# topling/toplingdb

Hardware: NVIDIA H100
Metric: compaction_input_kv_MB_per_s (higher is better)
Workload: dtype u8

## Files before the change

toplingdb_b200/csrc/encode.cu:

```cuda
#include "bloom_rules.h"
#include "common.cuh"
#include "gp_rules.h"
#include "kernels.h"
#include "scan.cuh"

namespace b200c {

constexpr int kTT = kEncTile;
constexpr int kW = kEncTile + kEncHalo;
constexpr int kEncThreads = 256;

__global__ void __launch_bounds__(256)
encode_sizes_kernel(KeyCols m, const unsigned long long* __restrict__ n_dev, uint32_t* __restrict__ esz, uint8_t* __restrict__ eshared,
                    TileStat* __restrict__ tstat, unsigned long long* __restrict__ tprefix, uint32_t* __restrict__ min_s1) {
  const uint64_t n = *n_dev;
  const uint64_t ntiles = (n + kEncTile - 1) / kEncTile;
  uint32_t mn = 0xffffffffu, mxs = 0;
  __shared__ unsigned long long red[5];
  __shared__ uint32_t s_mn, s_mx;
  if (threadIdx.x == 0) {
    s_mn = 0xffffffffu;
    s_mx = 0;
  }
  for (uint64_t tile = blockIdx.x; tile < ntiles; tile += gridDim.x) {
    if (threadIdx.x < 5) red[threadIdx.x] = threadIdx.x == 3 ? ~0ull : 0ull;
    __syncthreads();
    const uint64_t t0 = tile * kEncTile, t1 = (t0 + kEncTile) < n ? (t0 + kEncTile) : n;
    unsigned long long kb = 0, vb = 0, nd = 0, smin = ~0ull, smax = 0;
    constexpr int kB = 4;
    for (uint64_t ib = t0; ib < t1; ib += (uint64_t)kB * blockDim.x) {
      ulonglong2 c[kB], pc[kB];
      uint64_t ctr[kB], ptr_[kB];
      uint32_t cm[kB], pm[kB];
      const unsigned lane = threadIdx.x & 31;
#pragma unroll
      for (int q = 0; q < kB; q++) {
        const uint64_t i = ib + (uint64_t)q * blockDim.x + threadIdx.x;
        c[q] = make_ulonglong2(0, 0);
        pc[q] = make_ulonglong2(0, 0);
        ctr[q] = ptr_[q] = 0;
        cm[q] = pm[q] = 0;
        if (i < t1) {
          c[q] = m.pfx[i];
          ctr[q] = m.tr[i];
          cm[q] = m.meta[i];
          if (lane == 0 && i > 0) {
            pc[q] = m.pfx[i - 1];
            ptr_[q] = m.tr[i - 1];
            pm[q] = m.meta[i - 1];
          }
        }
      }
#pragma unroll
      for (int q = 0; q < kB; q++) {
        const uint64_t i = ib + (uint64_t)q * blockDim.x + threadIdx.x;
        const uint64_t nx = __shfl_up_sync(0xffffffffu, c[q].x, 1), ny = __shfl_up_sync(0xffffffffu, c[q].y, 1);
        const uint64_t nt = __shfl_up_sync(0xffffffffu, ctr[q], 1);
        const uint32_t nm = __shfl_up_sync(0xffffffffu, cm[q], 1);
        if (lane != 0) {
          pc[q] = make_ulonglong2(nx, ny);
          ptr_[q] = nt;
          pm[q] = nm;
        }
        if (i < t1) {
          const uint32_t ulen = meta_ulen(cm[q]), vs = meta_vlen(cm[q]), ks = ulen + 8;
          const uint32_t sh = i > 0 ? shared_prefix(c[q].x, c[q].y, ulen, ctr[q], pc[q].x, pc[q].y, meta_ulen(pm[q]), ptr_[q]) : 0;
          const uint32_t s1 = entry_size(sh, ks, vs);
          esz[i] = s1;
          eshared[i] = (uint8_t)sh;
          mn = s1 < mn ? s1 : mn;
          mxs = s1 > mxs ? s1 : mxs;
          kb += ks;
          vb += vs;
          nd += is_deletion_type((uint32_t)(ctr[q] & 0xff));
          const uint64_t sq = ctr[q] >> 8;
          smin = sq < smin ? sq : smin;
          smax = sq > smax ? sq : smax;
        }
      }
    }
#pragma unroll
    for (int d = 16; d; d >>= 1) {
      kb += __shfl_xor_sync(0xffffffffu, kb, d);
      vb += __shfl_xor_sync(0xffffffffu, vb, d);
      nd += __shfl_xor_sync(0xffffffffu, nd, d);
      const unsigned long long a = __shfl_xor_sync(0xffffffffu, smin, d), b = __shfl_xor_sync(0xffffffffu, smax, d);
      smin = a < smin ? a : smin;
      smax = b > smax ? b : smax;
    }
    if ((threadIdx.x & 31) == 0) {
      atomicAdd(&red[0], kb);
      atomicAdd(&red[1], vb);
      atomicAdd(&red[2], nd);
      atomicMin(&red[3], smin);
      atomicMax(&red[4], smax);
    }
    __syncthreads();
    if (threadIdx.x == 0) {
      tstat[tile] = TileStat{red[0], red[1], red[2], red[3], red[4]};
      tprefix[tile] = t1;
    }
    __syncthreads();
  }
  mn = __reduce_min_sync(0xffffffffu, mn);
  mxs = __reduce_max_sync(0xffffffffu, mxs);
  __syncthreads();
  if ((threadIdx.x & 31) == 0) {
    atomicMin(&s_mn, mn);
    atomicMax(&s_mx, mxs);
  }
  __syncthreads();
  if (threadIdx.x == 0 && s_mn != 0xffffffffu) {
    atomicMin(min_s1, s_mn);
    atomicMax(min_s1 + 1, s_mx);
  }
}

template <typename PT>
struct Window {
  PT P[kW + 1];
  uint32_t Q[kW];
  uint64_t ws[33];
  uint32_t wlen;
  uint32_t at_end;
  uint32_t smax;
};

template <typename PT>
__device__ void build_window(Window<PT>& w, const KeyCols& m, const uint32_t* esz, const uint8_t* eshared, uint64_t n, uint64_t tile,
                             uint32_t R) {
  const uint64_t wstart = tile * (uint64_t)kTT;
  const uint32_t wlen = (uint32_t)((n - wstart) < (uint64_t)kW ? (n - wstart) : (uint64_t)kW);
  uint32_t mx = 0;
  if (threadIdx.x == 0) w.smax = 0;
  constexpr int kBatch = 8;
  for (uint32_t jb = 0; jb < wlen; jb += kBatch * kEncThreads) {
    uint32_t s1v[kBatch], shv[kBatch], mtv[kBatch];
#pragma unroll
    for (int i = 0; i < kBatch; i++) {
      const uint32_t j = jb + i * kEncThreads + threadIdx.x;
      s1v[i] = shv[i] = mtv[i] = 0;
      if (j < wlen) {
        s1v[i] = esz[wstart + j];
        shv[i] = eshared[wstart + j];
        mtv[i] = m.meta[wstart + j];
      }
    }
#pragma unroll
    for (int i = 0; i < kBatch; i++) {
      const uint32_t j = jb + i * kEncThreads + threadIdx.x;
      if (j < wlen) {
        const uint32_t sh = shv[i], ks = meta_ulen(mtv[i]) + 8;
        const uint32_t d = 1u + varint_len32(ks) + sh - varint_len32(sh) - varint_len32(ks - sh);
        w.Q[j] = d;
        w.P[j + 1] = (PT)s1v[i];
        mx = s1v[i] + d > mx ? s1v[i] + d : mx;
      }
    }
  }
  __syncthreads();
  constexpr int kPer = ((kW + kEncThreads - 1) / kEncThreads) | 1;
  const uint32_t j0 = threadIdx.x * kPer;
  uint64_t loc[kPer], sum = 0;
#pragma unroll
  for (int i = 0; i < kPer; i++) {
    const uint32_t j = j0 + i;
    loc[i] = j < wlen ? w.P[j + 1] : 0;
    sum += loc[i];
  }
#pragma unroll
  for (int d = 16; d; d >>= 1) {
    uint32_t o = __shfl_xor_sync(0xffffffffu, mx, d);
    mx = o > mx ? o : mx;
  }
  uint64_t ex = block_excl_scan64(sum, nullptr, w.ws);
  if ((threadIdx.x & 31) == 0) atomicMax(&w.smax, mx);
#pragma unroll
  for (int i = 0; i < kPer; i++) {
    uint32_t j = j0 + i;
    if (j <= wlen && j <= (uint32_t)kW) w.P[j] = (PT)ex;
    ex += loc[i];
  }
  if (threadIdx.x == 0) {
    w.wlen = wlen;
    w.at_end = (wstart + wlen == n);
  }
  __syncthreads();
  if ((R & (R - 1)) == 0 && R <= 32 && kEncThreads % R == 0) {
    const uint32_t c = threadIdx.x & (R - 1), part = threadIdx.x / R, nparts = kEncThreads / R;
    const uint32_t per_class = (wlen + R - 1) / R;
    const uint32_t chunk = (per_class + nparts - 1) / nparts;
    const uint32_t first = part * chunk;
    uint32_t sum = 0;
    for (uint32_t i = 0; i < chunk; i++) {
      const uint32_t j = c + R * (first + i);
      if (j < wlen) sum += w.Q[j];
    }
    __shared__ uint32_t part_sum[kEncThreads];
    part_sum[threadIdx.x] = sum;
    __syncthreads();
    uint32_t run = 0;
    for (uint32_t q = 0; q < part; q++) run += part_sum[c + R * q];
    for (uint32_t i = 0; i < chunk; i++) {
      const uint32_t j = c + R * (first + i);
      if (j < wlen) {
        run += w.Q[j];
        w.Q[j] = run;
      }
    }
    __syncthreads();
  } else {
    for (uint32_t off = R; off < wlen; off <<= 1) {
      uint32_t add[kPer];
#pragma unroll
      for (int i = 0; i < kPer; i++) {
        uint32_t j = j0 + i;
        add[i] = (j < wlen && j >= off) ? w.Q[j - off] : 0;
      }
      __syncthreads();
#pragma unroll
      for (int i = 0; i < kPer; i++) {
        uint32_t j = j0 + i;
        if (j < wlen) w.Q[j] += add[i];
      }
      __syncthreads();
    }
  }
}

struct CutParams {
  uint32_t BS, LIM, R, rshift;
};
__host__ __device__ __forceinline__ CutParams make_cut(uint32_t bs, uint32_t lim, uint32_t r) {
  CutParams c{bs, lim, r, 32};
  if ((r & (r - 1)) == 0) {
    uint32_t sft = 0;
    while ((1u << sft) < r) sft++;
    c.rshift = sft;
  }
  return c;
}
__device__ __forceinline__ uint32_t div_r(uint32_t x, const CutParams& cp) { return cp.rshift < 32 ? x >> cp.rshift : x / cp.R; }
template <typename PT>
struct BlockStart {
  uint32_t a;
  PT pa;
  uint32_t qa;
};
template <typename PT>
__device__ __forceinline__ BlockStart<PT> block_start(const Window<PT>& w, uint32_t a, const CutParams& cp) {
  BlockStart<PT> s;
  s.a = a;
  s.pa = w.P[a];
  s.qa = a >= cp.R ? w.Q[a - cp.R] : 0u;
  return s;
}
template <typename PT>
__device__ __forceinline__ PT blk_payload(const Window<PT>& w, const BlockStart<PT>& s, uint32_t b, const CutParams& cp) {
  const uint32_t nrm1 = div_r(b - 1 - s.a, cp);
  const uint32_t last = s.a + cp.R * nrm1;
  const uint32_t q = w.Q[last] - s.qa;
  return (PT)(w.P[b] - s.pa) + (PT)q + (PT)(4u * (nrm1 + 1) + 4u);
}
template <typename PT>
__device__ __forceinline__ PT blk_payload(const Window<PT>& w, uint32_t a, uint32_t b, const CutParams& cp) {
  return blk_payload(w, block_start(w, a, cp), b, cp);
}
template <typename PT>
__device__ __forceinline__ uint32_t next_block(const Window<PT>& w, uint32_t a, const CutParams& cp, uint32_t hint, PT* pay_out) {
  const uint32_t wlen = w.wlen;
  const BlockStart<PT> bs = block_start(w, a, cp);
  PT thr = (PT)(cp.BS - 1);
  if (cp.LIM) {
    thr = (PT)cp.LIM;
    const uint64_t guard = (uint64_t)w.smax + 7;
    if (cp.BS > guard && cp.BS - guard - 1 > thr) thr = (PT)(cp.BS - guard - 1);
  }
  uint32_t lo = a + 1, hi = wlen + 1;
  PT ec_hi = 0;
  if (hint > a + 1 && hint <= wlen) {
    const PT ph = blk_payload(w, bs, hint, cp);
    uint32_t step = 1;
    if (ph > thr) {
      hi = hint;
      ec_hi = ph;
      while (hi - lo >= step) {
        const uint32_t mid = hi - step;
        const PT pm = blk_payload(w, bs, mid, cp);
        if (pm > thr) {
          hi = mid;
          ec_hi = pm;
          step <<= 1;
        } else {
          lo = mid + 1;
          break;
        }
      }
    } else {
      lo = hint + 1;
      while (lo + step - 1 <= wlen) {
        const uint32_t mid = lo + step - 1;
        const PT pm = blk_payload(w, bs, mid, cp);
        if (pm > thr) {
          hi = mid;
          ec_hi = pm;
          break;
// ... 6 lines not shown
  while (lo < hi) {
    const uint32_t mid = (lo + hi) >> 1;
    const PT pm = blk_payload(w, bs, mid, cp);
    if (pm > thr) {
      hi = mid;
      ec_hi = pm;
    } else {
      lo = mid + 1;
    }
  }
  if (lo >= wlen) {
    if (!w.at_end) return 0xffffffffu;
    *pay_out = blk_payload(w, bs, wlen, cp);
    return wlen;
  }
  PT ec = ec_hi;
  uint32_t m = lo - a;
  uint32_t mr = cp.rshift < 32 ? (m & (cp.R - 1)) : (m % cp.R);
  for (uint32_t b = lo; b < wlen; b++) {
    if (ec >= cp.BS) {
      *pay_out = ec;
      return b;
    }
    const PT s1 = (PT)(w.P[b + 1] - w.P[b]);
    const bool at_restart = mr == 0;
    const PT d = at_restart ? (PT)(w.Q[b] - (b >= cp.R ? w.Q[b - cp.R] : 0u)) : (PT)0;
    if (cp.LIM) {
      const PT dfull = at_restart ? d : (PT)(w.Q[b] - (b >= cp.R ? w.Q[b - cp.R] : 0u));
      if (ec + s1 + dfull + 3 + (at_restart ? 4 : 0) > cp.BS) {
        *pay_out = ec;
        return b;
      }
    }
    ec += s1 + (at_restart ? d + 4 : 0);
    mr = mr + 1 == cp.R ? 0 : mr + 1;
  }
  if (!w.at_end) return 0xffffffffu;
  *pay_out = ec;
  return wlen;
}

constexpr int kEncGroup = kEncGroupTiles;
__device__ __forceinline__ TileRow ldcg_row(const TileRow* p) {
  const uint4 v = __ldcg(reinterpret_cast<const uint4*>(p));
  TileRow r;
  r.exit = v.x;
  r.nblk = v.y;
  r.bytes = (uint64_t)v.z | ((uint64_t)v.w << 32);
  return r;
}
static_assert(sizeof(TileRow) == 16, "TileRow is moved as one 16-byte vector");
__device__ void compose_group(const EncodeWork& wk, uint64_t n, uint64_t g, uint64_t t0, uint64_t t1, uint32_t hc) {
  const uint64_t gstart = t0 * (uint64_t)kTT;
  for (uint32_t c = threadIdx.x; c < hc; c += blockDim.x) {
    uint64_t x = gstart + c, bytes = 0;
    uint32_t nb = 0;
    bool bad = false;
    for (uint64_t t = t0; t < t1 && x < n; t++) {
      const uint64_t tstart = t * (uint64_t)kTT, tend = (tstart + kTT) < n ? (tstart + kTT) : n;
      if (x >= tend) continue;
      const uint64_t cc = x - tstart;
      if (cc >= hc) {
        bad = true;
        break;
      }
      const TileRow r = ldcg_row(&wk.rows[t * hc + cc]);
      if (r.exit == 0xffffffffu) {
        bad = true;
        break;
      }
      x = tstart + r.exit;
      nb += r.nblk;
      bytes += r.bytes;
    }
    TileRow o;
    o.exit = bad ? 0xffffffffu : (uint32_t)(x - gstart);
    o.nblk = nb;
    o.bytes = bytes;
    wk.grows[g * hc + c] = o;
  }
}

template <typename PT>
struct TablesSmem {
  Window<PT> w;
  uint16_t nxt[kTT];
  uint32_t disk[kTT];
};
template <typename PT>
__global__ void __launch_bounds__(kEncThreads, sizeof(PT) == 4 ? 3 : 2)
encode_tables_kernel(KeyCols m, EncodeParams ep, EncodeWork wk, uint64_t n, uint32_t hc, uint16_t* __restrict__ g_nxt,
                     uint32_t* __restrict__ g_disk, uint32_t* __restrict__ err) {
  extern __shared__ __align__(16) uint8_t smem_raw[];
  TablesSmem<PT>& s = *reinterpret_cast<TablesSmem<PT>*>(smem_raw);
  const uint64_t tile = blockIdx.x, wstart = tile * (uint64_t)kTT;
  const CutParams cp = make_cut(ep.block_size, ep.block_size_limit, ep.restart_interval);
  build_window(s.w, m, wk.esz, wk.eshared, n, tile, cp.R);
  const uint32_t tl = s.w.wlen < (uint32_t)kTT ? s.w.wlen : (uint32_t)kTT;
  {
    constexpr int kPer = kTT / kEncThreads;
    const PT total = s.w.P[s.w.wlen];
    const uint32_t per_block = total ? (uint32_t)(((uint64_t)ep.block_size * s.w.wlen) / total) : 0;
    uint32_t prev_pos = 0, prev_b = 0;
    for (int i = 0; i < kPer; i++) {
      const uint32_t j = threadIdx.x * kPer + ((i + threadIdx.x) & (kPer - 1));
      if (j >= tl) continue;
      uint32_t hint = j + 1 + per_block;
      if (prev_b) hint = prev_b + j - prev_pos;
      if (hint > s.w.wlen) hint = s.w.wlen;
      PT pay = 0;
      uint32_t b = next_block(s.w, j, cp, hint, &pay);
      prev_pos = j;
      prev_b = b == 0xffffffffu ? 0 : b;
      uint16_t nx = 0xffff;
      uint32_t dk = 0;
      if (b != 0xffffffffu) {
        nx = (uint16_t)b;
        const uint64_t pay5 = (uint64_t)pay + 5;
        dk = pay5 > 0xffffffffull ? 0xffffffffu : (uint32_t)pay5;
      }
      s.nxt[j] = nx;
      s.disk[j] = dk;
    }
  }
  __syncthreads();
  for (uint32_t j = threadIdx.x; j < tl; j += kEncThreads) {
    g_nxt[wstart + j] = s.nxt[j];
    g_disk[wstart + j] = s.disk[j];
  }
  __syncthreads();
  for (uint32_t c = threadIdx.x; c < hc; c += kEncThreads) {
    uint32_t x = c, nb = 0;
    uint64_t bytes = 0;
    bool bad = false;
    while (x < tl) {
      uint32_t y = s.nxt[x];
      if (y == 0xffff || y <= x) {
        bad = true;
        break;
      }
      bytes += s.disk[x];
      nb++;
      x = y;
    }
    TileRow r;
    r.exit = bad ? 0xffffffffu : x;
    r.nblk = nb;
    r.bytes = bytes;
    wk.rows[tile * hc + c] = r;
  }
  (void)err;
  __threadfence();
  __syncthreads();
  __shared__ uint32_t s_last;
  const uint64_t g = tile / kEncGroupTiles, ntiles = (n + kTT - 1) / kTT;
  const uint64_t t0 = g * kEncGroupTiles, t1 = (t0 + kEncGroupTiles) < ntiles ? (t0 + kEncGroupTiles) : ntiles;
  if (threadIdx.x == 0) s_last = atomicAdd(&wk.gdone[g], 1u) + 1 == (uint32_t)(t1 - t0);
  __syncthreads();
  if (!s_last) return;
  __threadfence();
  compose_group(wk, n, g, t0, t1, hc);
  __threadfence();
  __syncthreads();
  if (threadIdx.x == 0) atomicExch(&wk.gready[g], 1u);
}

struct WalkState {
  uint64_t a;
  uint64_t blk;
  uint64_t foff;
  uint64_t f_first_entry, f_first_blk;
  uint32_t f;
};
__device__ __forceinline__ void close_file(FileRec* files, WalkState& st, uint64_t end_entry, uint32_t* err) {
  if (files == nullptr) return;
  if (st.f >= kMaxOutFiles) {
    atomicOr(err, kErrInternal);
    return;
  }
  FileRec& fr = files[st.f];
  fr.first_entry = st.f_first_entry;
  fr.n_entries = end_entry - st.f_first_entry;
  fr.first_block = st.f_first_blk;
  fr.n_blocks = st.blk - st.f_first_blk;
  fr.data_size = st.foff;
  fr.index_size = 0;
  fr.raw_key_size = fr.raw_value_size = fr.num_deletions = 0;
  fr.smallest_seq = ~0ull;
  fr.largest_seq = 0;
  fr.index_has_seq = 0;
  fr.filter_entries = fr.filter_bytes = 0;
}
__device__ __forceinline__ uint64_t single_entry_block_bytes(const KeyCols& m, const EncodeWork& wk, uint64_t y) {
  uint32_t sh = wk.eshared[y], ks = meta_ulen(m.meta[y]) + 8;
  uint64_t s0 = (uint64_t)wk.esz[y] + 1u + varint_len32(ks) + sh - varint_len32(sh) - varint_len32(ks - sh);
  return s0 + 4 + 4 + 5;
}
__device__ uint64_t truncated_block_bytes(const KeyCols& m, const EncodeWork& wk, uint32_t R, uint64_t a, uint64_t e) {
  uint64_t sum = 0;
  for (uint64_t j0 = a; j0 < e; j0 += 8) {
    uint32_t s1[8], sh[8], mt[8];
#pragma unroll
    for (int q = 0; q < 8; q++) {
      const uint64_t j = j0 + q;
      s1[q] = sh[q] = mt[q] = 0;
      if (j < e) {
        s1[q] = wk.esz[j];
        sh[q] = wk.eshared[j];
        mt[q] = m.meta[j];
      }
    }
#pragma unroll
    for (int q = 0; q < 8; q++) {
      const uint64_t j = j0 + q;
      if (j < e) {
        sum += s1[q];
        if ((j - a) % R == 0) {
          const uint32_t ks = meta_ulen(mt[q]) + 8;
          sum += 1u + varint_len32(ks) + sh[q] - varint_len32(sh[q]) - varint_len32(ks - sh[q]);
        }
      }
    }
  }
  const uint64_t nrest = (e - a + R - 1) / R;
// ... 184 lines not shown
          const uint64_t cc = st.a - tstart;
          TileRow r;
          r.exit = 0xffffffffu;
          if (cc < hc) r = tcache[(t - cta) * hc + cc];
          const bool table_ok = cc < hc && r.exit != 0xffffffffu;
          const bool cut = !table_ok || (ep.output_level != 0 && st.foff + r.bytes >= ep.max_output_file_size) || tstart + r.exit >= n ||
                           next_ev <= tstart + r.exit;
          if (cut) {
            req = 1;
            req_idx = t;
            break;
          }
          st.a = tstart + r.exit;
          st.blk += r.nblk;
          st.foff += r.bytes;
          continue;
        }
        if (cg >= ngroups) {
          fin = 1;
          break;
        }
        const uint64_t gg = cg, t0 = gg * kEncGroup, gstart = t0 * (uint64_t)kTT;
        const uint64_t t1 = (t0 + kEncGroup) < ntiles ? (t0 + kEncGroup) : ntiles;
        const uint64_t gend = (t1 * (uint64_t)kTT) < n ? (t1 * (uint64_t)kTT) : n;
        if (st.a < gend && !(gg >= cga && gg < cga + cgn)) {
          req = 2;
          req_idx = gg;
          break;
        }
        TileState gs{st.a, st.blk, st.foff, st.f, 0};
        wk.gstate[gg] = gs;
        wk.gflag[gg] = 0;
        cg++;
        if (st.a >= gend) continue;
        const uint64_t cc = st.a - gstart;
        TileRow r;
        r.exit = 0xffffffffu;
        if (cc < hc) r = gcache[(gg - cga) * hc + cc];
        const bool table_ok = cc < hc && r.exit != 0xffffffffu;
        const bool cut = !table_ok || (ep.output_level != 0 && st.foff + r.bytes >= ep.max_output_file_size) || gstart + r.exit >= n ||
                         next_ev <= gstart + r.exit;
        if (cut) {
          wk.gflag[gg] = 1;
          ct = t0;
          ctend = t1;
          continue;
        }
        st.a = gstart + r.exit;
        st.blk += r.nblk;
        st.foff += r.bytes;
      }
      s.st = st;
      s.g = cg;
      s.t = ct;
      s.tend = ctend;
      s.req = req;
      s.req_idx = req_idx;
      if (fin) s.done = 1;
    }
    __syncthreads();
    const uint32_t req = s.req;
    const uint64_t ridx = s.req_idx;
    uint32_t done = s.done;
    if (req == 2 || req == 3) {
      const uint64_t total = req == 2 ? ngroups : s.tend;
      uint32_t cnt = (uint32_t)((total - ridx) < cache_rows ? (total - ridx) : cache_rows);
      if (req == 2) {
        if (threadIdx.x == 0) {
          volatile uint32_t* rdy = wk.gready;
          if (first_wait) {
            unsigned long long t0, t1;
            asm volatile("mov.u64 %0, %globaltimer;" : "=l"(t0));
            while (rdy[ridx] == 0) {
              __nanosleep(256);
              asm volatile("mov.u64 %0, %globaltimer;" : "=l"(t1));
              if (t1 - t0 > timeout_ns) {
                s.done = 2;
                break;
              }
            }
          } else {
            while (rdy[ridx] == 0) __nanosleep(256);
          }
          uint32_t have = 1;
          while (have < cnt && rdy[ridx + have] != 0) have++;
          s.refill = have;
          __threadfence();
        }
        __syncthreads();
        if (s.done == 2) return;
        first_wait = false;
        cnt = s.refill;
      }
      const uint4* src = reinterpret_cast<const uint4*>((req == 2 ? wk.grows : wk.rows) + ridx * hc);
      uint4* dst = reinterpret_cast<uint4*>(req == 2 ? gcache : tcache);
      coop_copy_cg<uint4, 8>(dst, src, cnt * hc);
      if (threadIdx.x == 0) {
        if (req == 2) {
          s.ga = ridx;
          s.gn = cnt;
        } else {
          s.ta = ridx;
          s.tn = cnt;
        }
      }
    } else if (req == 1) {
      const uint64_t tstart = ridx * (uint64_t)kTT;
      const uint32_t tl = (uint32_t)(((tstart + kTT) < n ? (tstart + kTT) : n) - tstart);
      const uint32_t c0 = (uint32_t)(s.st.a > tstart ? (s.st.a - tstart) & ~7ull : 0);
      const uint32_t c1 = (tl + 7u) & ~7u;
      coop_copy_cg<uint4, 4>(reinterpret_cast<uint4*>(s.nxt + c0), reinterpret_cast<const uint4*>(wk.nxt + tstart + c0), (c1 - c0) / 8);
      coop_copy_cg<uint4, 8>(reinterpret_cast<uint4*>(s.disk + c0), reinterpret_cast<const uint4*>(wk.disk + tstart + c0), (c1 - c0) / 4);
      __syncthreads();
      if (ep.gp.n == 0) {
        for (uint32_t i = c0 + threadIdx.x; i < tl; i += blockDim.x) s.nd[i] = ((uint64_t)s.nxt[i] << 32) | s.disk[i];
        __syncthreads();
      }
      if (threadIdx.x == 0) {
        WalkState st = s.st;
        GpState g = s.gp;
        bool chased = true;
        if (ep.gp.n) {
          chased = chase_tile<1>(s.nxt, s.disk, tstart, tl, n, ep, m, wk, st, wk.files, nullptr, 0, err, &g);
        } else {
          const uint32_t nd_base = (uint32_t)__cvta_generic_to_shared(s.nd);
          const uint64_t left = n - tstart;
          const uint32_t nlocal = left < 0xffffull ? (uint32_t)left : 0xffffu;
          const bool cut_files = ep.output_level != 0;
          const uint64_t fmax = ep.max_output_file_size;
          uint32_t x = (uint32_t)(st.a - tstart);
          uint64_t foff = st.foff, blk = st.blk;
          while (x < tl) {
            for (;;) {
              uint64_t v;
              asm volatile("ld.shared.u64 %0, [%1];" : "=l"(v) : "r"(nd_base + 8u * x));
              const uint32_t yr = (uint32_t)(v >> 32), d = (uint32_t)v;
              const uint64_t nf = foff + d;
              if (yr <= x || yr >= nlocal || (cut_files && nf >= fmax)) break;
              foff = nf;
              blk++;
              x = yr;
              if (x >= tl) break;
            }
            if (x >= tl) break;
            st.a = tstart + x;
            st.foff = foff;
            st.blk = blk;
            chased = chase_tile<0>(s.nxt, s.disk, tstart, x + 1, n, ep, m, wk, st, wk.files, nullptr, 0, err);
            if (!chased || st.a >= n) break;
            x = (uint32_t)(st.a - tstart);
            foff = st.foff;
            blk = st.blk;
          }
          if (chased && st.a < n && x >= tl && st.a < tstart + x) {
            st.a = tstart + x;
            st.foff = foff;
            st.blk = blk;
          }
        }
        s.gp = g;
        if (!chased) {
          atomicOr(err, kErrBlockTooLong);
          s.done = 1;
        }
        s.st = st;
      }
      __syncthreads();
      done = s.done;
    }
    __syncthreads();
    if (done) break;
  }
  if (threadIdx.x == 0) {
    wk.totals[0] = s.st.blk;
    wk.totals[1] = s.st.f;
    TileState ts{n, s.st.blk, 0, s.st.f, 0};
    for (uint64_t t = s.t; t < s.tend; t++) wk.tstate[t] = ts;
    for (uint64_t gg = s.g; gg < ngroups; gg++) {
      wk.gstate[gg] = ts;
      wk.gflag[gg] = 0;
    }
    __threadfence();
    if (attempt == 1) atomicExch(sflag, 1u);
  }
}

__global__ void encode_tilestate_kernel(EncodeWork wk, uint64_t n, uint64_t ntiles, uint32_t hc, uint32_t* __restrict__ err) {
  const uint64_t g = blockIdx.x * (uint64_t)blockDim.x + threadIdx.x;
  const uint64_t ngroups = (ntiles + kEncGroup - 1) / kEncGroup;
  if (g >= ngroups || wk.gflag[g]) return;
  const TileState gs = wk.gstate[g];
  uint64_t a = gs.entry, blk = gs.blk, foff = gs.file_off;
  const uint64_t t0 = g * kEncGroup, t1 = (t0 + kEncGroup) < ntiles ? (t0 + kEncGroup) : ntiles;
  for (uint64_t t = t0; t < t1; t++) {
    const uint64_t tstart = t * (uint64_t)kTT, tend = (tstart + kTT) < n ? (tstart + kTT) : n;
    TileState ts{a < n ? a : n, blk, foff, gs.file_idx, 0};
    wk.tstate[t] = ts;
    if (a >= n || a >= tend) continue;
    const uint64_t cc = a - tstart;
    if (cc >= hc) {
      atomicOr(err, kErrBlockTooLong);
      return;
    }
    const TileRow r = wk.rows[t * hc + cc];
    if (r.exit == 0xffffffffu) {
      atomicOr(err, kErrBlockTooLong);
      return;
    }
    a = tstart + r.exit;
    blk += r.nblk;
    foff += r.bytes;
  }
}

struct BlistSmem {
  uint16_t nxt[kTT];
  uint32_t disk[kTT];
  uint8_t is_start[kTT];
  uint64_t ws[33];
  uint32_t serial;
};
__global__ void __launch_bounds__(kEncThreads)
encode_blocklist_kernel(KeyCols m, EncodeParams ep, EncodeWork wk, uint64_t n, uint64_t nblk_cap, uint32_t* __restrict__ err) {
  __shared__ BlistSmem s;
  const uint64_t tile = blockIdx.x, tstart = tile * (uint64_t)kTT;
  const uint64_t tend = (tstart + kTT) < n ? (tstart + kTT) : n;
  const uint32_t tl = (uint32_t)(tend - tstart);
  const TileState ts = wk.tstate[tile];
  if (ts.entry >= tend) return;
  for (uint32_t j = threadIdx.x; j < tl; j += kEncThreads) {
    s.nxt[j] = wk.nxt[tstart + j];
    s.disk[j] = wk.disk[tstart + j];
    s.is_start[j] = 0;
  }
  __syncthreads();
  if (threadIdx.x == 0) {
    uint32_t x = (uint32_t)(ts.entry - tstart);
    uint64_t bytes = 0;
    bool bad = false, ends = false;
    while (x < tl) {
      uint32_t y = s.nxt[x];
      if (y == 0xffff || y <= x) {
        bad = true;
        break;
      }
      s.is_start[x] = 1;
      bytes += s.disk[x];
      if (tstart + y >= n) ends = true;
      x = y;
    }
    if (bad) atomicOr(err, kErrBlockTooLong);
    bool gp_cut = false;
    if (ep.gp.n && !bad) {
      const uint32_t nc = *ep.gp_ncuts;
      uint32_t lo = 0, hi = nc;
      while (lo < hi) {
        const uint32_t mid = (lo + hi) >> 1;
        if (ep.gp_cuts[mid].entry <= ts.entry) lo = mid + 1;
        else hi = mid;
      }
      gp_cut = lo < nc && ep.gp_cuts[lo].entry <= tstart + x;
    }
    s.serial = bad ? 2 : ((ends || gp_cut || (ep.output_level != 0 && ts.file_off + bytes >= ep.max_output_file_size)) ? 1 : 0);
    if (s.serial == 1) {
      WalkState st;
      st.a = ts.entry;
      st.blk = ts.blk;
      st.foff = ts.file_off;
      st.f = ts.file_idx;
      st.f_first_entry = 0;
      st.f_first_blk = 0;
      const bool chased = ep.gp.n ? chase_tile<2>(s.nxt, s.disk, tstart, tl, n, ep, m, wk, st, nullptr, wk.blocks, nblk_cap, err)
                                  : chase_tile<0>(s.nxt, s.disk, tstart, tl, n, ep, m, wk, st, nullptr, wk.blocks, nblk_cap, err);
      if (!chased) atomicOr(err, kErrBlockTooLong);
    }
  }
  __syncthreads();
  if (s.serial != 0) return;
  constexpr int kPer = kTT / kEncThreads;
  const uint32_t j0 = threadIdx.x * kPer;
  uint32_t cnt = 0;
  uint64_t bytes = 0;
#pragma unroll
  for (int i = 0; i < kPer; i++) {
    uint32_t j = j0 + i;
    if (j < tl && s.is_start[j]) {
      cnt++;
      bytes += s.disk[j];
    }
  }
  uint64_t packed = ((uint64_t)cnt << 48) | bytes;
  uint64_t ex = block_excl_scan64(packed, nullptr, s.ws);
  uint64_t r = ts.blk + (ex >> 48), off = ts.file_off + (ex & ((1ull << 48) - 1));
#pragma unroll
  for (int i = 0; i < kPer; i++) {
    uint32_t j = j0 + i;
    if (j < tl && s.is_start[j]) {
      if (r < nblk_cap) wk.blocks[r] = BlockRec{tstart + j, off, ts.file_idx, (uint32_t)(s.nxt[j] - j)};
      r++;
      off += s.disk[j];
    }
  }
}

__device__ __forceinline__ uint64_t index_entries_bytes(const EncodeWork& wk, uint64_t b0, uint64_t nb) {
  return wk.idx_eoff[b0 + nb - 1] + wk.idx_esz[b0 + nb - 1] - wk.idx_eoff[b0];
}

__global__ void encode_filestats_kernel(KeyCols m, EncodeWork wk, uint32_t nfiles) {
  const uint32_t f = blockIdx.x;
  if (f >= nfiles) return;
  const uint64_t f0 = wk.files[f].first_entry, f1 = f0 + wk.files[f].n_entries;
  __shared__ unsigned long long red[5];
  if (threadIdx.x < 5) red[threadIdx.x] = threadIdx.x == 3 ? ~0ull : 0ull;
  __syncthreads();
  const unsigned long long kVal = (1ull << 62) - 1;
// ... 985 lines not shown
                        uint32_t cksum, uint8_t* const* out_base, uint64_t* contrib, const uint64_t* contrib_off, cudaStream_t st) {
  if (n == 0 || nfiles == 0) return;
  const int probes = bloom_num_probes((int)millibits);
  static PerDeviceFlag attr;
  const uint64_t dev_bit = attr.bit_of_current_device();
  const int smem = (int)kBloomSliceBytes + 16 + (kBloomThreads / 32) * kBloomStage * 8;
  if (!attr.is_set(dev_bit)) {
    cudaFuncSetAttribute(bloom_slices_kernel, cudaFuncAttributeMaxDynamicSharedMemorySize, smem);
    attr.set(dev_bit);
  }
  const unsigned slices = (max_filter_bytes + kBloomSliceBytes - 1) / kBloomSliceBytes;
  bloom_slices_kernel<<<dim3(slices ? slices : 1, nfiles), kBloomThreads, smem, st>>>(hashes, files, nfiles, probes, out_base);
  if (cksum == 4) file_block_contrib_kernel<<<dim3(32, nfiles), 256, 0, st>>>(files, nfiles, kFilterBlock, out_base, contrib, contrib_off);
  file_block_trailer_kernel<<<(nfiles + 3) / 4, 128, 0, st>>>(files, nfiles, kFilterBlock, cksum, out_base, contrib, contrib_off);
}

__global__ void gp_rank_kernel(KeyCols m, const GpKey* __restrict__ smallest, const GpKey* __restrict__ largest, uint32_t n,
                               uint64_t* __restrict__ lo, uint64_t* __restrict__ eq, uint64_t* __restrict__ hi) {
  const uint32_t i = blockIdx.x * blockDim.x + threadIdx.x;
  if (i >= n) return;
  auto bound = [&](const GpKey& k, bool upper) -> uint64_t {
    uint64_t a = 0, b = m.n;
    while (a < b) {
      const uint64_t mid = a + ((b - a) >> 1);
      const ulonglong2 p = m.pfx[mid];
      const int c = ukey_cmp(p.x, p.y, meta_ulen(m.meta[mid]), k.hi, k.lo, k.ulen);
      if (c < 0 || (upper && c == 0)) a = mid + 1;
      else b = mid;
    }
    return a;
  };
  lo[i] = bound(smallest[i], false);
  eq[i] = bound(largest[i], false);
  hi[i] = bound(largest[i], true);
}
void launch_gp_ranks(KeyCols m, const GpKey* smallest, const GpKey* largest, uint32_t n, uint64_t* lo, uint64_t* eq, uint64_t* hi,
                     cudaStream_t st) {
  if (n) gp_rank_kernel<<<(n + 63) / 64, 64, 0, st>>>(m, smallest, largest, n, lo, eq, hi);
}

__global__ void scatter_tails_kernel(const TailCopy* __restrict__ recs, const uint8_t* __restrict__ staged, uint8_t* __restrict__ out) {
  const TailCopy r = recs[blockIdx.x];
  for (uint32_t i = threadIdx.x; i < r.len; i += blockDim.x) out[r.dst_off + i] = staged[r.src_off + i];
}

__global__ void gather_small_kernel(const uint64_t* __restrict__ small, uint32_t small_words, const FileRec* __restrict__ files,
                                    const uint64_t* __restrict__ nfiles_dev, uint64_t* __restrict__ dst) {
  const uint32_t t = blockIdx.x * blockDim.x + threadIdx.x, nt = gridDim.x * blockDim.x;
  for (uint32_t i = t; i < small_words; i += nt) dst[i] = small[i];
  if (files) {
    uint64_t n = *nfiles_dev;
    if (n > kMaxOutFiles) n = kMaxOutFiles;
    const uint64_t words = n * (sizeof(FileRec) / 8);
    const uint64_t* src = reinterpret_cast<const uint64_t*>(files);
    for (uint64_t i = t; i < words; i += nt) dst[small_words + i] = src[i];
  }
}
static_assert(sizeof(FileRec) % 8 == 0, "FileRec is copied word-wise");

void launch_gather_small(const uint64_t* small, uint32_t small_bytes, const FileRec* files, const uint64_t* nfiles_dev, uint8_t* dst,
                         cudaStream_t st) {
  gather_small_kernel<<<files ? 8 : 1, 256, 0, st>>>(small, small_bytes / 8, files, nfiles_dev, reinterpret_cast<uint64_t*>(dst));
}
__global__ void copy_small_kernel(const uint8_t* __restrict__ src, uint8_t* __restrict__ dst, uint32_t n) {
  for (uint32_t i = threadIdx.x; i < n; i += blockDim.x) dst[i] = src[i];
}
void launch_copy_small(const void* src, void* dst, uint32_t n, cudaStream_t st) {
  if (n) copy_small_kernel<<<1, 256, 0, st>>>(static_cast<const uint8_t*>(src), static_cast<uint8_t*>(dst), n);
}
void launch_scatter_tails(const TailCopy* recs, uint32_t n, const uint8_t* staged, uint8_t* out, cudaStream_t st) {
  if (n) scatter_tails_kernel<<<n, 256, 0, st>>>(recs, staged, out);
}
void launch_encode_sizes(KeyCols m, const unsigned long long* n_dev, EncodeWork w, unsigned long long* tprefix_out, uint64_t n_cap,
                         int sms, cudaStream_t st) {
  if (n_cap == 0) return;
  const uint64_t tiles = (n_cap + kEncTile - 1) / kEncTile;
  encode_sizes_kernel<<<(unsigned)(tiles < (unsigned)sms * 8 ? tiles : (unsigned)sms * 8), 256, 0, st>>>(m, n_dev, w.esz, w.eshared, w.tstat, tprefix_out, w.min_s1);
}
void launch_encode_tables(KeyCols m, EncodeParams ep, EncodeWork w, uint64_t ntiles, uint32_t hc, uint32_t max_s1, uint32_t* err,
                          cudaStream_t st) {
  if (ntiles == 0) return;
  static PerDeviceFlag attr;
  const uint64_t dev_bit = attr.bit_of_current_device();
  if (!attr.is_set(dev_bit)) {
    cudaFuncSetAttribute(encode_tables_kernel<uint32_t>, cudaFuncAttributeMaxDynamicSharedMemorySize, (int)sizeof(TablesSmem<uint32_t>));
    cudaFuncSetAttribute(encode_tables_kernel<uint64_t>, cudaFuncAttributeMaxDynamicSharedMemorySize, (int)sizeof(TablesSmem<uint64_t>));
    attr.set(dev_bit);
  }
  if (((uint64_t)max_s1 + 64) * (uint64_t)(kW + 1) < (1ull << 32))
    encode_tables_kernel<uint32_t><<<(unsigned)ntiles, kEncThreads, sizeof(TablesSmem<uint32_t>), st>>>(m, ep, w, m.n, hc, w.nxt, w.disk, err);
  else
    encode_tables_kernel<uint64_t><<<(unsigned)ntiles, kEncThreads, sizeof(TablesSmem<uint64_t>), st>>>(m, ep, w, m.n, hc, w.nxt, w.disk, err);
}
void launch_encode_stitch(KeyCols m, EncodeParams ep, EncodeWork w, uint64_t ntiles, uint32_t hc, uint32_t* err, uint32_t attempt,
                          uint32_t* sflag, cudaStream_t st, uint64_t* launches) {
  if (ntiles == 0) return;
  static PerDeviceFlag attr;
  const uint64_t dev_bit = attr.bit_of_current_device();
  constexpr size_t kSolo = 200 * 1024;
  if (!attr.is_set(dev_bit)) {
    cudaFuncSetAttribute(encode_stitch_kernel, cudaFuncAttributeMaxDynamicSharedMemorySize, (int)kSolo);
    attr.set(dev_bit);
  }
  const size_t fixed = (sizeof(StitchSmem) + 15) & ~(size_t)15;
  uint32_t cache_bytes = 16 * 1024;
  while (cache_bytes < hc * (uint32_t)sizeof(TileRow)) cache_bytes *= 2;
  size_t smem = fixed + 2 * (size_t)cache_bytes;
  if (attempt == 1) {
    const uint32_t big = (uint32_t)(((kSolo - fixed) / 2) & ~(size_t)15);
    if (big > cache_bytes) cache_bytes = big;
    smem = kSolo;
  }
  encode_stitch_kernel<<<1, kEncThreads, smem, st>>>(m, ep, w, m.n, ntiles, hc, cache_bytes, err, attempt, sflag, 300000u);
  if (launches) *launches += 1;
}
void launch_encode_tilestate(KeyCols m, EncodeWork w, uint64_t ntiles, uint32_t hc, uint32_t* err, cudaStream_t st, uint64_t* launches) {
  if (ntiles == 0) return;
  const uint64_t ngroups = (ntiles + kEncGroup - 1) / kEncGroup;
  encode_tilestate_kernel<<<(unsigned)((ngroups + 63) / 64), 64, 0, st>>>(w, m.n, ntiles, hc, err);
  if (launches) *launches += 1;
}
void launch_encode_blocklist(KeyCols m, EncodeParams ep, EncodeWork w, uint64_t ntiles, uint64_t nblk_cap, uint32_t* err,
                             cudaStream_t st) {
  if (ntiles == 0) return;
  encode_blocklist_kernel<<<(unsigned)ntiles, kEncThreads, 0, st>>>(m, ep, w, m.n, nblk_cap, err);
}
void launch_encode_filestats(KeyCols m, EncodeWork w, uint32_t nfiles, cudaStream_t st) {
  if (m.n == 0 || nfiles == 0) return;
  encode_filestats_kernel<<<nfiles, 256, 0, st>>>(m, w, nfiles);
}
constexpr uint32_t kEmitMaxSmem = 224 * 1024;
uint32_t encode_emit_slice(uint32_t block_size) {
  uint32_t s = block_size + block_size / 4 + 512;
  s = (s + 255) & ~255u;
  if (s < 5632) s = 5632;
  if (s > 24 * 1024) s = 24 * 1024;
  return s;
}
static_assert(kEmitWarps * (24 * 1024 + 2 * kStageBytes) <= kEmitMaxSmem, "the largest slots and their column stages fit one CTA");
void launch_encode_emit(KeyCols m, EncodeParams ep, EncodeWork w, uint64_t nblocks, uint8_t* const* out_base, uint64_t data_bytes,
                        uint32_t* err, int sms, cudaStream_t st) {
  if (nblocks == 0) return;
  static PerDeviceFlag attr;
  const uint64_t dev_bit = attr.bit_of_current_device();
  if (!attr.is_set(dev_bit)) {
    cudaFuncSetAttribute(encode_emit_kernel, cudaFuncAttributeMaxDynamicSharedMemorySize, kEmitMaxSmem);
    cudaFuncSetAttribute(encode_emit_long_kernel, cudaFuncAttributeMaxDynamicSharedMemorySize, kEmitMaxSmem);
    attr.set(dev_bit);
  }
  const bool long_entries = data_bytes > 64 * m.n;
  const int warps = long_entries ? kEmitLongWarps : kEmitWarps, ctas = long_entries ? kEmitLongCtasPerSm : kEmitCtasPerSm;
  const uint32_t slot = encode_emit_slice(ep.block_size);
  const size_t smem = (size_t)warps * (slot + (long_entries ? 0 : 2 * kStageBytes));
  int per_sm = 0;
  cudaOccupancyMaxActiveBlocksPerMultiprocessor(&per_sm, long_entries ? (const void*)encode_emit_long_kernel : (const void*)encode_emit_kernel,
                                                warps * 32, smem);
  if (per_sm < 1) per_sm = 1;
  if (per_sm > ctas) per_sm = ctas;
  const uint64_t want = (nblocks + warps - 1) / warps;
  const uint64_t cap = (uint64_t)sms * per_sm;
  const unsigned grid = (unsigned)(want < cap ? want : cap);
  if (long_entries) encode_emit_long_kernel<<<grid, warps * 32, smem, st>>>(m, ep, w, nblocks, out_base, slot, err);
  else encode_emit_kernel<<<grid, warps * 32, smem, st>>>(m, ep, w, nblocks, out_base, slot, err);
}
static unsigned index_grid(uint64_t nblocks, int sms) {
  const uint64_t g = (nblocks + 255) / 256;
  return (unsigned)(g < (uint64_t)sms * 8 ? g : (uint64_t)sms * 8);
}
void launch_encode_index_size(KeyCols m, EncodeParams ep, EncodeWork w, uint64_t nblocks, int sms, cudaStream_t st, uint64_t* launches) {
  if (nblocks == 0) return;
  const unsigned g = index_grid(nblocks, sms);
  encode_index_sep_kernel<<<g, 256, 0, st>>>(m, w, nblocks);
  encode_index_size_kernel<<<g, 256, 0, st>>>(w, nblocks, ep.format_version);
  exclusive_scan<uint32_t>(w.idx_esz, w.idx_eoff, nblocks, w.scan_tmp, nullptr, st, launches);
  if (launches) *launches += 2;
// ... 20 lines not shown
```

Measured before the change: 275,100.

## Size encode window by halo count, drop smem disk array, vectorize blocklist loads

The encode-tables window length now depends on the runtime halo count (hc), not a fixed maximum. The per-entry disk array is removed from shared memory and recomputed from the prefix sums where it is needed, and the min-blocks hint is raised so more blocks fit per SM. The blocklist kernel loads nxt and disk with 16-byte vector loads, and the stitch refill readiness scan is spread across threads instead of run serially by one. In exchange, block payload sizes are recomputed in the hc chain walk, registers may spill under the tighter launch bounds, and the loop trip counts become dynamic.

```diff
diff --git a/toplingdb_b200/csrc/encode.cu b/toplingdb_b200/csrc/encode.cu
--- a/toplingdb_b200/csrc/encode.cu
+++ b/toplingdb_b200/csrc/encode.cu
@@ -7,7 +7,6 @@
 namespace b200c {
 
 constexpr int kTT = kEncTile;
-constexpr int kW = kEncTile + kEncHalo;
 constexpr int kEncThreads = 256;
 
 __global__ void __launch_bounds__(256)
@@ -116,24 +115,33 @@
   }
 }
 
+constexpr uint32_t kEncHaloAlign = 64;
+constexpr int kWinPerMax = ((kEncTile + kEncHalo + kEncThreads) / kEncThreads) | 1;
+__host__ __device__ constexpr uint32_t enc_window_len(uint32_t hc) {
+  const uint32_t halo = (hc + kEncHaloAlign - 1) / kEncHaloAlign * kEncHaloAlign;
+  return (uint32_t)kEncTile + (halo < (uint32_t)kEncHalo ? halo : (uint32_t)kEncHalo);
+}
 template <typename PT>
 struct Window {
-  PT P[kW + 1];
-  uint32_t Q[kW];
-  uint64_t ws[33];
+  PT* P;
+  uint32_t* Q;
   uint32_t wlen;
   uint32_t at_end;
   uint32_t smax;
 };
 
 template <typename PT>
-__device__ void build_window(Window<PT>& w, const KeyCols& m, const uint32_t* esz, const uint8_t* eshared, uint64_t n, uint64_t tile,
-                             uint32_t R) {
+__device__ __forceinline__ void build_window(Window<PT>& w, const KeyCols& m, const uint32_t* esz, const uint8_t* eshared, uint64_t n,
+                                             uint64_t tile, uint32_t wmax, uint32_t R) {
+  __shared__ uint64_t ws[33];
+  __shared__ uint32_t s_smax;
   const uint64_t wstart = tile * (uint64_t)kTT;
-  const uint32_t wlen = (uint32_t)((n - wstart) < (uint64_t)kW ? (n - wstart) : (uint64_t)kW);
+  const uint32_t wlen = (uint32_t)((n - wstart) < (uint64_t)wmax ? (n - wstart) : (uint64_t)wmax);
+  w.wlen = wlen;
+  w.at_end = (wstart + wlen == n);
   uint32_t mx = 0;
-  if (threadIdx.x == 0) w.smax = 0;
-  constexpr int kBatch = 8;
+  if (threadIdx.x == 0) s_smax = 0;
+  constexpr int kBatch = 9;
   for (uint32_t jb = 0; jb < wlen; jb += kBatch * kEncThreads) {
     uint32_t s1v[kBatch], shv[kBatch], mtv[kBatch];
 #pragma unroll
@@ -159,13 +167,14 @@
     }
   }
   __syncthreads();
-  constexpr int kPer = ((kW + kEncThreads - 1) / kEncThreads) | 1;
-  const uint32_t j0 = threadIdx.x * kPer;
-  uint64_t loc[kPer], sum = 0;
-#pragma unroll
-  for (int i = 0; i < kPer; i++) {
+  const uint32_t per = ((wmax + kEncThreads) / kEncThreads) | 1;
+  const uint32_t j0 = threadIdx.x * per;
+  uint32_t loc[kWinPerMax];
+  uint64_t sum = 0;
+#pragma unroll
+  for (int i = 0; i < kWinPerMax; i++) {
     const uint32_t j = j0 + i;
-    loc[i] = j < wlen ? w.P[j + 1] : 0;
+    loc[i] = (i < per && j < wlen) ? (uint32_t)w.P[j + 1] : 0u;
     sum += loc[i];
   }
 #pragma unroll
@@ -173,19 +182,16 @@
     uint32_t o = __shfl_xor_sync(0xffffffffu, mx, d);
     mx = o > mx ? o : mx;
   }
-  uint64_t ex = block_excl_scan64(sum, nullptr, w.ws);
-  if ((threadIdx.x & 31) == 0) atomicMax(&w.smax, mx);
-#pragma unroll
-  for (int i = 0; i < kPer; i++) {
-    uint32_t j = j0 + i;
-    if (j <= wlen && j <= (uint32_t)kW) w.P[j] = (PT)ex;
+  uint64_t ex = block_excl_scan64(sum, nullptr, ws);
+  if ((threadIdx.x & 31) == 0) atomicMax(&s_smax, mx);
+#pragma unroll
+  for (int i = 0; i < kWinPerMax; i++) {
+    const uint32_t j = j0 + i;
+    if (i < per && j <= wlen) w.P[j] = (PT)ex;
     ex += loc[i];
   }
-  if (threadIdx.x == 0) {
-    w.wlen = wlen;
-    w.at_end = (wstart + wlen == n);
-  }
   __syncthreads();
+  w.smax = s_smax;
   if ((R & (R - 1)) == 0 && R <= 32 && kEncThreads % R == 0) {
     const uint32_t c = threadIdx.x & (R - 1), part = threadIdx.x / R, nparts = kEncThreads / R;
     const uint32_t per_class = (wlen + R - 1) / R;
@@ -211,17 +217,17 @@
     __syncthreads();
   } else {
     for (uint32_t off = R; off < wlen; off <<= 1) {
-      uint32_t add[kPer];
-#pragma unroll
-      for (int i = 0; i < kPer; i++) {
-        uint32_t j = j0 + i;
-        add[i] = (j < wlen && j >= off) ? w.Q[j - off] : 0;
+      uint32_t add[kWinPerMax];
+#pragma unroll
+      for (int i = 0; i < kWinPerMax; i++) {
+        const uint32_t j = j0 + i;
+        add[i] = (i < per && j < wlen && j >= off) ? w.Q[j - off] : 0;
       }
       __syncthreads();
 #pragma unroll
-      for (int i = 0; i < kPer; i++) {
-        uint32_t j = j0 + i;
-        if (j < wlen) w.Q[j] += add[i];
+      for (int i = 0; i < kWinPerMax; i++) {
+        const uint32_t j = j0 + i;
+        if (i < per && j < wlen) w.Q[j] += add[i];
       }
       __syncthreads();
     }
@@ -394,64 +400,64 @@
 }
 
 template <typename PT>
-struct TablesSmem {
-  Window<PT> w;
-  uint16_t nxt[kTT];
-  uint32_t disk[kTT];
-};
+__device__ __forceinline__ uint32_t block_disk(const Window<PT>& w, uint32_t a, uint32_t b, const CutParams& cp) {
+  const uint64_t pay5 = (uint64_t)blk_payload(w, a, b, cp) + 5;
+  return pay5 > 0xffffffffull ? 0xffffffffu : (uint32_t)pay5;
+}
+
+__host__ __device__ constexpr size_t align16(size_t x) { return (x + 15) & ~(size_t)15; }
 template <typename PT>
-__global__ void __launch_bounds__(kEncThreads, sizeof(PT) == 4 ? 3 : 2)
-encode_tables_kernel(KeyCols m, EncodeParams ep, EncodeWork wk, uint64_t n, uint32_t hc, uint16_t* __restrict__ g_nxt,
+__host__ __device__ constexpr size_t tables_smem_bytes(uint32_t wmax) {
+  return align16(sizeof(PT) * ((size_t)wmax + 1)) + align16(4 * (size_t)wmax) + 2 * (size_t)kTT;
+}
+template <typename PT>
+__global__ void __launch_bounds__(kEncThreads, sizeof(PT) == 4 ? 4 : 3)
+encode_tables_kernel(KeyCols m, EncodeParams ep, EncodeWork wk, uint64_t n, uint32_t hc, uint32_t wmax, uint16_t* __restrict__ g_nxt,
                      uint32_t* __restrict__ g_disk, uint32_t* __restrict__ err) {
   extern __shared__ __align__(16) uint8_t smem_raw[];
-  TablesSmem<PT>& s = *reinterpret_cast<TablesSmem<PT>*>(smem_raw);
+  Window<PT> w;
+  w.P = reinterpret_cast<PT*>(smem_raw);
+  w.Q = reinterpret_cast<uint32_t*>(smem_raw + align16(sizeof(PT) * ((size_t)wmax + 1)));
+  uint16_t* nxt = reinterpret_cast<uint16_t*>(smem_raw + align16(sizeof(PT) * ((size_t)wmax + 1)) + align16(4 * (size_t)wmax));
   const uint64_t tile = blockIdx.x, wstart = tile * (uint64_t)kTT;
   const CutParams cp = make_cut(ep.block_size, ep.block_size_limit, ep.restart_interval);
-  build_window(s.w, m, wk.esz, wk.eshared, n, tile, cp.R);
-  const uint32_t tl = s.w.wlen < (uint32_t)kTT ? s.w.wlen : (uint32_t)kTT;
+  build_window(w, m, wk.esz, wk.eshared, n, tile, wmax, cp.R);
+  const uint32_t tl = w.wlen < (uint32_t)kTT ? w.wlen : (uint32_t)kTT;
   {
     constexpr int kPer = kTT / kEncThreads;
-    const PT total = s.w.P[s.w.wlen];
-    const uint32_t per_block = total ? (uint32_t)(((uint64_t)ep.block_size * s.w.wlen) / total) : 0;
+    const PT total = w.P[w.wlen];
+    const uint32_t per_block = total ? (uint32_t)(((uint64_t)ep.block_size * w.wlen) / total) : 0;
     uint32_t prev_pos = 0, prev_b = 0;
     for (int i = 0; i < kPer; i++) {
       const uint32_t j = threadIdx.x * kPer + ((i + threadIdx.x) & (kPer - 1));
       if (j >= tl) continue;
       uint32_t hint = j + 1 + per_block;
       if (prev_b) hint = prev_b + j - prev_pos;
-      if (hint > s.w.wlen) hint = s.w.wlen;
+      if (hint > w.wlen) hint = w.wlen;
       PT pay = 0;
-      uint32_t b = next_block(s.w, j, cp, hint, &pay);
+      uint32_t b = next_block(w, j, cp, hint, &pay);
       prev_pos = j;
       prev_b = b == 0xffffffffu ? 0 : b;
-      uint16_t nx = 0xffff;
-      uint32_t dk = 0;
-      if (b != 0xffffffffu) {
-        nx = (uint16_t)b;
-        const uint64_t pay5 = (uint64_t)pay + 5;
-        dk = pay5 > 0xffffffffull ? 0xffffffffu : (uint32_t)pay5;
-      }
-      s.nxt[j] = nx;
-      s.disk[j] = dk;
+      nxt[j] = b == 0xffffffffu ? (uint16_t)0xffff : (uint16_t)b;
     }
   }
   __syncthreads();
   for (uint32_t j = threadIdx.x; j < tl; j += kEncThreads) {
-    g_nxt[wstart + j] = s.nxt[j];
-    g_disk[wstart + j] = s.disk[j];
-  }
-  __syncthreads();
+    const uint32_t y = nxt[j];
+    g_nxt[wstart + j] = (uint16_t)y;
+    g_disk[wstart + j] = y == 0xffff ? 0u : block_disk(w, j, y, cp);
+  }
   for (uint32_t c = threadIdx.x; c < hc; c += kEncThreads) {
     uint32_t x = c, nb = 0;
     uint64_t bytes = 0;
     bool bad = false;
     while (x < tl) {
-      uint32_t y = s.nxt[x];
+      uint32_t y = nxt[x];
       if (y == 0xffff || y <= x) {
         bad = true;
         break;
       }
-      bytes += s.disk[x];
+      bytes += block_disk(w, x, y, cp);
       nb++;
       x = y;
     }
@@ -802,13 +808,14 @@
           } else {
             while (rdy[ridx] == 0) __nanosleep(256);
           }
-          uint32_t have = 1;
-          while (have < cnt && rdy[ridx + have] != 0) have++;
-          s.refill = have;
-          __threadfence();
+          s.refill = cnt;
         }
         __syncthreads();
         if (s.done == 2) return;
+        for (uint32_t i = 1 + threadIdx.x; i < cnt; i += blockDim.x)
+          if (reinterpret_cast<volatile const uint32_t*>(wk.gready)[ridx + i] == 0) atomicMin(&s.refill, i);
+        __threadfence();
+        __syncthreads();
         first_wait = false;
         cnt = s.refill;
       }
@@ -942,16 +949,40 @@
 };
 __global__ void __launch_bounds__(kEncThreads)
 encode_blocklist_kernel(KeyCols m, EncodeParams ep, EncodeWork wk, uint64_t n, uint64_t nblk_cap, uint32_t* __restrict__ err) {
-  __shared__ BlistSmem s;
+  __shared__ __align__(16) BlistSmem s;
   const uint64_t tile = blockIdx.x, tstart = tile * (uint64_t)kTT;
   const uint64_t tend = (tstart + kTT) < n ? (tstart + kTT) : n;
   const uint32_t tl = (uint32_t)(tend - tstart);
   const TileState ts = wk.tstate[tile];
   if (ts.entry >= tend) return;
-  for (uint32_t j = threadIdx.x; j < tl; j += kEncThreads) {
-    s.nxt[j] = wk.nxt[tstart + j];
-    s.disk[j] = wk.disk[tstart + j];
-    s.is_start[j] = 0;
+  {
+    constexpr int kNv = kTT / 8 / kEncThreads, kDv = kTT / 4 / kEncThreads;
+    const uint32_t nv = (tl + 7) / 8, dv = (tl + 3) / 4;
+    const uint4* gn = reinterpret_cast<const uint4*>(wk.nxt + tstart);
+    const uint4* gd = reinterpret_cast<const uint4*>(wk.disk + tstart);
+    uint4 a[kNv], b[kDv];
+#pragma unroll
+    for (int k = 0; k < kNv; k++) {
+      const uint32_t i = k * kEncThreads + threadIdx.x;
+      if (i < nv) a[k] = gn[i];
+    }
+#pragma unroll
+    for (int k = 0; k < kDv; k++) {
+      const uint32_t i = k * kEncThreads + threadIdx.x;
+      if (i < dv) b[k] = gd[i];
+    }
+#pragma unroll
+    for (int k = 0; k < kNv; k++) {
+      const uint32_t i = k * kEncThreads + threadIdx.x;
+      if (i < nv) reinterpret_cast<uint4*>(s.nxt)[i] = a[k];
+    }
+#pragma unroll
+    for (int k = 0; k < kDv; k++) {
+      const uint32_t i = k * kEncThreads + threadIdx.x;
+      if (i < dv) reinterpret_cast<uint4*>(s.disk)[i] = b[k];
+    }
+    static_assert(kTT == 16 * kEncThreads, "one 16-byte vector of is_start per thread");
+    reinterpret_cast<uint4*>(s.is_start)[threadIdx.x] = make_uint4(0, 0, 0, 0);
   }
   __syncthreads();
   if (threadIdx.x == 0) {
@@ -2103,15 +2134,17 @@
   if (ntiles == 0) return;
   static PerDeviceFlag attr;
   const uint64_t dev_bit = attr.bit_of_current_device();
+  constexpr uint32_t kWMax = kEncTile + kEncHalo;
   if (!attr.is_set(dev_bit)) {
-    cudaFuncSetAttribute(encode_tables_kernel<uint32_t>, cudaFuncAttributeMaxDynamicSharedMemorySize, (int)sizeof(TablesSmem<uint32_t>));
-    cudaFuncSetAttribute(encode_tables_kernel<uint64_t>, cudaFuncAttributeMaxDynamicSharedMemorySize, (int)sizeof(TablesSmem<uint64_t>));
+    cudaFuncSetAttribute(encode_tables_kernel<uint32_t>, cudaFuncAttributeMaxDynamicSharedMemorySize, (int)tables_smem_bytes<uint32_t>(kWMax));
+    cudaFuncSetAttribute(encode_tables_kernel<uint64_t>, cudaFuncAttributeMaxDynamicSharedMemorySize, (int)tables_smem_bytes<uint64_t>(kWMax));
     attr.set(dev_bit);
   }
-  if (((uint64_t)max_s1 + 64) * (uint64_t)(kW + 1) < (1ull << 32))
-    encode_tables_kernel<uint32_t><<<(unsigned)ntiles, kEncThreads, sizeof(TablesSmem<uint32_t>), st>>>(m, ep, w, m.n, hc, w.nxt, w.disk, err);
+  const uint32_t wmax = enc_window_len(hc);
+  if (((uint64_t)max_s1 + 64) * (uint64_t)(wmax + 1) < (1ull << 32))
+    encode_tables_kernel<uint32_t><<<(unsigned)ntiles, kEncThreads, tables_smem_bytes<uint32_t>(wmax), st>>>(m, ep, w, m.n, hc, wmax, w.nxt, w.disk, err);
   else
-    encode_tables_kernel<uint64_t><<<(unsigned)ntiles, kEncThreads, sizeof(TablesSmem<uint64_t>), st>>>(m, ep, w, m.n, hc, w.nxt, w.disk, err);
+    encode_tables_kernel<uint64_t><<<(unsigned)ntiles, kEncThreads, tables_smem_bytes<uint64_t>(wmax), st>>>(m, ep, w, m.n, hc, wmax, w.nxt, w.disk, err);
 }
 void launch_encode_stitch(KeyCols m, EncodeParams ep, EncodeWork w, uint64_t ntiles, uint32_t hc, uint32_t* err, uint32_t attempt,
                           uint32_t* sflag, cudaStream_t st, uint64_t* launches) {
```

Result: faster. 281,500, median of 6 (+2.3%).
